# SamuelGong/FLASHE

Measured on AMD Instinct MI355X. Metric: ciphertexts/sec (enc+agg+dec), 1e7-elem vector; achieved HBM GB/s fraction, higher is better.
Workload: dtype u128

## Files before the change

flashe_amd/csrc/abi.hip:

```cpp
#include "ctx.h"
#include "blockpool.h"

#include <algorithm>
#include <cstdarg>
#include <cstdio>
#include <cstdlib>
#include <cmath>
#include <cstring>
#include <mutex>
#include <new>
#include <string>
#include <vector>

using namespace flashe;

namespace {

struct AesTables {
    uint8_t sbox[256];
    uint32_t te0[256];
    AesTables()
    {
        uint8_t alog[256], lg[256];
        uint8_t x = 1;
// ... 816 lines not shown
        idx[c] = first_idx + static_cast<uint32_t>(c);
        if (idx[c] < first_idx) return fail(ctx, FLASHE_EINVAL, "the cohort's cipher indices wrap around 2^32");
    }
    if ((rc = check_double_idx(ctx, FLASHE_SCHEME_DOUBLE, idx.data(), n_clients))) return rc;
    if (n == 0) return FLASHE_OK;
    for (int c = 0; c < n_clients; c++)
        if (!mask_dev[c] || (reinterpret_cast<uintptr_t>(mask_dev[c]) & 3u)) return fail(ctx, FLASHE_EINVAL, "vector %d: null or not 4-byte aligned", c);
    LaunchEnv env = ctx->env;
    env.elem32 = 1;
    const std::vector<const uint64_t *> none(static_cast<size_t>(n_clients), nullptr);
    return batch_shares(ctx, n_clients, [&](int v0, int nv) {
        return launch_prf_batch(env, iter, true, nv, idx.data() + v0, none.data() + v0, 1, reinterpret_cast<uint64_t *const *>(mask_dev + v0), n, n_jobs);
    });
}

int flashe_encrypt_batch_sum_u32_dev(flashe_ctx *ctx, uint32_t iter, int scheme, uint64_t n, uint32_t n_jobs, int n_vec, const uint32_t *idx,
                                     const uint32_t *const *pt_dev, uint32_t *const *ct_dev, uint32_t *sum_out_dev)
{
    CHECK_CTX(ctx);
    if (n && !sum_out_dev) return fail(ctx, FLASHE_EINVAL, "flashe_encrypt_batch_sum_u32_dev: null sum_out_dev");
    if (reinterpret_cast<uintptr_t>(sum_out_dev) & 3u) return fail(ctx, FLASHE_EINVAL, "sum_out_dev must be 4-byte aligned");
    if (n && ct_dev) { if (int rc = check_sum_apart(ctx, sum_out_dev, n_vec, pt_dev, ct_dev)) return rc; }
    if (scheme == FLASHE_SCHEME_DOUBLE && n && n_vec > 0 && n_vec <= kMaxUniformBatch && idx && pt_dev && ct_dev) {
        int rc = check_u32(ctx, n, n_jobs);
        if (rc || (rc = check_double_idx(ctx, scheme, idx, n_vec))) return rc;
        bool ok = true;
        for (int v = 0; v < n_vec && ok; v++)
            ok = pt_dev[v] && ct_dev[v] && !((reinterpret_cast<uintptr_t>(pt_dev[v]) | reinterpret_cast<uintptr_t>(ct_dev[v])) & 3u) && (v == 0 || idx[v] == idx[v - 1] + 1u);
        if (ok) {
            LaunchEnv env = ctx->env;
            env.elem32 = 1;
            std::vector<uint32_t> sidx(idx, idx + n_vec);
            sidx.push_back(idx[n_vec - 1] + 1u);
            PrfChain ch{sidx.data(), n_vec, false, 0, n, reinterpret_cast<const uint64_t *const *>(pt_dev), 1, reinterpret_cast<uint64_t *const *>(ct_dev)};
            ch.sum_out_dev = reinterpret_cast<uint64_t *>(sum_out_dev);
            const hipError_t e = launch_prf_chains(env, iter, 1, &ch, n, n_jobs);
            if (e == hipSuccess) return FLASHE_OK;
            if (e != hipErrorNotSupported) HIP_TRY(ctx, e);
        }
    }
    int rc = flashe_encrypt_batch_u32_dev(ctx, iter, scheme, n, n_jobs, n_vec, idx, pt_dev, ct_dev);
    if (rc || n == 0) return rc;
    if (n_vec == 0) { HIP_TRY(ctx, hipMemsetAsync(sum_out_dev, 0, n * 4, ctx->env.stream)); return FLASHE_OK; }
    return flashe_aggregate_elem_u32_dev(ctx, n_vec, ct_dev, n, sum_out_dev);
}

int flashe_aggregate_decrypt_u32_dev(flashe_ctx *ctx, uint32_t iter, const uint32_t *add_idx, int n_add, const uint32_t *minus_idx, int n_minus,
                                     uint64_t n, uint32_t n_jobs, uint64_t first, uint64_t count, int C, const uint32_t *const *cts_dev,
                                     void *agg_out_dev, void *out_dev, int out_elem_bytes)
{
    CHECK_CTX(ctx);
    if (C < 1 || C > kMaxOps || !cts_dev || (count && !out_dev)) return fail(ctx, FLASHE_EINVAL, "aggregate_decrypt_u32: bad arguments (C = %d, at most %d)", C, kMaxOps);
    if (out_elem_bytes != 4 && out_elem_bytes != 8) return fail(ctx, FLASHE_EINVAL, "out_elem_bytes must be 4 or 8");
    if (n_add != 1 || n_minus < 0 || n_minus > 1 || !add_idx || (n_minus && !minus_idx))
        return fail(ctx, FLASHE_EINVAL, "aggregate_decrypt_u32: one add and at most one minus prefix (widen the vectors for prefix lists)");
    int rc = check_u32(ctx, n, n_jobs);
    if (rc) return rc;
    rc = check_range(ctx, n, first, count);
    if (rc) return rc;
    if (count == 0) return FLASHE_OK;
    if ((rc = check_operands(ctx, C, cts_dev, 4))) return rc;
    const uintptr_t need = static_cast<uintptr_t>(out_elem_bytes - 1);
    if ((reinterpret_cast<uintptr_t>(out_dev) | reinterpret_cast<uintptr_t>(agg_out_dev)) & need) return fail(ctx, FLASHE_EINVAL, "outputs must be %d-byte aligned", out_elem_bytes);
    LaunchEnv env = ctx->env;
    env.elem32 = 1;
    if (C == 1 && !agg_out_dev && out_elem_bytes == 4 && n_minus == 1) {
        const uint32_t sidx[2] = {add_idx[0], minus_idx[0]};
        const uint64_t *in1 = reinterpret_cast<const uint64_t *>(cts_dev[0]);
        uint64_t *out1 = static_cast<uint64_t *>(out_dev);
        PrfChain ch{sidx, 1, false, first, count, &in1, 1, &out1};
        const hipError_t e = launch_prf_chains(env, iter, 1, &ch, n, n_jobs);
        if (e == hipSuccess) return FLASHE_OK;
        if (e != hipErrorNotSupported) HIP_TRY(ctx, e);
    }
    HIP_TRY(ctx, launch_small_reduce_decrypt(env, iter, add_idx[0], n_minus == 1, n_minus ? minus_idx[0] : 0u, n, n_jobs, first, count, C,
                                             reinterpret_cast<const uint64_t *const *>(cts_dev), static_cast<uint64_t *>(agg_out_dev),
                                             static_cast<uint64_t *>(out_dev), out_elem_bytes));
    return FLASHE_OK;
}

int flashe_aggregate_elem_u32_dev(flashe_ctx *ctx, int C, const uint32_t *const *cts_dev, uint64_t n, uint32_t *out_dev)
// ... 17 lines not shown

int flashe_widen_u32_dev(flashe_ctx *ctx, uint64_t n, const uint32_t *in_dev, uint64_t *out_dev)
{
    CHECK_CTX(ctx);
    if (n && (!in_dev || !out_dev)) return fail(ctx, FLASHE_EINVAL, "widen_u32: null vector");
    HIP_TRY(ctx, launch_widen_u32(ctx->env, n, in_dev, out_dev));
    return FLASHE_OK;
}

int flashe_narrow_u32_dev(flashe_ctx *ctx, uint64_t n, const uint64_t *in_dev, uint32_t *out_dev)
{
    CHECK_CTX(ctx);
    if (n && (!in_dev || !out_dev)) return fail(ctx, FLASHE_EINVAL, "narrow_u32: null vector");
    HIP_TRY(ctx, launch_narrow_u32(ctx->env, n, in_dev, out_dev));
    return FLASHE_OK;
}

static uint64_t *chain_dmask_begin(flashe_ctx *ctx, uint64_t count)
{
    flashe_ctx::ChainDmask &s = ctx->chain_dmask;
    s.valid = false;
    if (!ctx->chain_dmask_on || ctx->capturing || ctx->limbs != 2 || count == 0) return nullptr;
    if (ensure(ctx, s.d, vec_bytes(ctx, count)) != FLASHE_OK) {
        (void)hipGetLastError();
        ctx->err.clear();
        return nullptr;
    }
    return static_cast<uint64_t *>(s.d.p);
}

static void chain_dmask_commit(flashe_ctx *ctx, uint32_t iter, const uint32_t *idx, int n_vec, uint64_t n, uint32_t n_jobs, uint64_t first,
                               uint64_t count)
{
    flashe_ctx::ChainDmask &s = ctx->chain_dmask;
    s.iter = iter; s.key_epoch = ctx->key_epoch; s.add_idx = idx[n_vec - 1] + 1u; s.minus_idx = idx[0];
    s.n = n; s.n_jobs = n_jobs; s.first = first; s.count = count;
    s.valid = true;
}

static const uint64_t *chain_dmask_match(const flashe_ctx *ctx, uint32_t iter, const uint32_t *add_idx, int n_add, const uint32_t *minus_idx,
                                         int n_minus, uint64_t n, uint32_t n_jobs, uint64_t first, uint64_t count)
{
    const flashe_ctx::ChainDmask &s = ctx->chain_dmask;
    if (!s.valid || ctx->capturing || n_add != 1 || n_minus != 1 || count == 0) return nullptr;
    if (add_idx[0] != s.add_idx || minus_idx[0] != s.minus_idx || iter != s.iter || ctx->key_epoch != s.key_epoch || n != s.n ||
        n_jobs != s.n_jobs)
        return nullptr;
    if (first < s.first || first - s.first > s.count || count > s.count - (first - s.first)) return nullptr;
    return static_cast<const uint64_t *>(s.d.p) + (first - s.first) * 2;
}

static int encrypt_batch_sum(flashe_ctx *ctx, uint32_t iter, int scheme, uint64_t n, uint32_t n_jobs, int n_vec, const uint32_t *idx,
                             const uint64_t *const *pt_dev, int pt_limbs, uint64_t *const *ct_dev, uint64_t *sum_out_dev, uint64_t *dec_out_dev,
                             bool *dec_done)
{
    if (!sum_out_dev && n && n_vec) return fail(ctx, FLASHE_EINVAL, "flashe_encrypt_batch_sum_dev: null sum_out_dev");
    if (n_vec > 0) { if (int rc = check_double_idx(ctx, scheme, idx, n_vec)) return rc; }
    if (n && n_vec) {
        if (int rc = check_sum_aligned(ctx, sum_out_dev)) return rc;
        if (int rc = check_sum_apart(ctx, sum_out_dev, n_vec, pt_dev, ct_dev)) return rc;
    }
    if (scheme == FLASHE_SCHEME_DOUBLE && n && n_vec > 0 && idx && pt_dev && ct_dev) {
        bool ok = true;
        for (int v = 0; v < n_vec && ok; v++) ok = pt_dev[v] && ct_dev[v];
        if (ok) {
            for (int v = 0; v < n_vec; v++) {
                int rc = check_prf_args(ctx, 1, scheme, n_jobs, ct_dev[v], pt_dev[v], pt_limbs);
                if (rc) return rc;
            }
            if (dec_out_dev && ctx->chain_dec_on) {
                const hipError_t e = launch_prf_batch_sum(ctx->env, iter, n_vec, idx, pt_dev, pt_limbs, ct_dev, sum_out_dev, n, n_jobs, 0, n, nullptr,
                                                          dec_out_dev);
                if (e == hipSuccess) { *dec_done = true; return FLASHE_OK; }
                if (e != hipErrorNotSupported) HIP_TRY(ctx, e);
            }
            uint64_t *const dmask = chain_dmask_begin(ctx, n);
            const hipError_t e = launch_prf_batch_sum(ctx->env, iter, n_vec, idx, pt_dev, pt_limbs, ct_dev, sum_out_dev, n, n_jobs, 0, n, dmask);
            if (e == hipSuccess) {
                if (dmask) chain_dmask_commit(ctx, iter, idx, n_vec, n, n_jobs, 0, n);
                return FLASHE_OK;
            }
            if (e != hipErrorNotSupported) HIP_TRY(ctx, e);
        }
    }
    int rc = flashe_encrypt_batch_dev(ctx, iter, scheme, n, n_jobs, n_vec, idx, pt_dev, pt_limbs, ct_dev);
    if (rc || n == 0) return rc;
    if (n_vec == 0) { HIP_TRY(ctx, hipMemsetAsync(sum_out_dev, 0, n * ctx->limbs * 8, ctx->env.stream)); return FLASHE_OK; }
    return flashe_aggregate_elem_dev(ctx, n_vec, ct_dev, n, sum_out_dev);
}

int flashe_encrypt_batch_sum_dev(flashe_ctx *ctx, uint32_t iter, int scheme, uint64_t n, uint32_t n_jobs, int n_vec, const uint32_t *idx,
                                 const uint64_t *const *pt_dev, int pt_limbs, uint64_t *const *ct_dev, uint64_t *sum_out_dev)
{
    CHECK_CTX(ctx);
// ... 171 lines not shown
    int rc = check_range(ctx, n, first, count);
    if (rc || (rc = check_double_idx(ctx, scheme, idx, n_vec))) return rc;
    if (n_jobs == 0) return fail(ctx, FLASHE_EINVAL, "n_jobs must be >= 1");
    if (ctx->env.prf_backend != PRF_AUTO && ctx->env.prf_backend != PRF_TABLE) return fail(ctx, FLASHE_EINVAL, "encrypt_batch_range runs on the table PRF only");
    for (int v = 0; v < n_vec; v++) {
        if (count && (!pt_dev[v] || !ct_dev[v])) return fail(ctx, FLASHE_EINVAL, "null vector %d", v);
        if (sum_out_dev && (ct_dev[v] == sum_out_dev || pt_dev[v] == sum_out_dev))
            return fail(ctx, FLASHE_EINVAL, "sum_out_dev must not be one of the plaintext or ciphertext vectors");
        rc = check_prf_args(ctx, 1, scheme, n_jobs, ct_dev[v], pt_dev[v], pt_limbs);
        if (rc) return rc;
    }
    if (sum_out_dev && (rc = check_sum_aligned(ctx, sum_out_dev))) return rc;
    if (count == 0) return FLASHE_OK;
    if (n_vec == 0) { if (sum_out_dev) HIP_TRY(ctx, hipMemsetAsync(sum_out_dev, 0, vec_bytes(ctx, count), ctx->env.stream)); return FLASHE_OK; }
    if (sum_out_dev && scheme == FLASHE_SCHEME_DOUBLE) {
        uint64_t *const dmask = chain_dmask_begin(ctx, count);
        const hipError_t e = launch_prf_batch_sum(ctx->env, iter, n_vec, idx, pt_dev, pt_limbs, ct_dev, sum_out_dev, n, n_jobs, first, count, dmask);
        if (e == hipSuccess) {
            if (dmask) chain_dmask_commit(ctx, iter, idx, n_vec, n, n_jobs, first, count);
            return FLASHE_OK;
        }
        if (e != hipErrorNotSupported) HIP_TRY(ctx, e);
    }
    rc = batch_shares(ctx, n_vec, [&](int v0, int nv) {
        return launch_prf_batch_range(ctx->env, iter, scheme == FLASHE_SCHEME_DOUBLE, nv, idx + v0, pt_dev + v0, pt_limbs, ct_dev + v0, n, n_jobs,
                                      first, count);
    });
    if (rc) return rc;
    if (sum_out_dev) return flashe_aggregate_elem_dev(ctx, n_vec, ct_dev, count, sum_out_dev);
    return FLASHE_OK;
}

int flashe_decrypt_range_dev(flashe_ctx *ctx, uint32_t iter, const uint32_t *add_idx, int n_add, const uint32_t *minus_idx,
                             int n_minus, uint64_t n, uint32_t n_jobs, uint64_t first, uint64_t count,
                             const uint64_t *in_dev, uint64_t *out_dev)
{
    CHECK_CTX(ctx);
    if (count && (!in_dev || !out_dev)) return fail(ctx, FLASHE_EINVAL, "null vector");
    int rc = check_prf_args(ctx, n_add, n_minus, n_jobs, out_dev, in_dev, ctx->limbs);
    if (rc || (rc = check_range(ctx, n, first, count))) return rc;
    if (n_add == 0 && n_minus == 0) {
        HIP_TRY(ctx, launch_combine(ctx->env, count, in_dev, ctx->limbs, nullptr, nullptr, out_dev));
        return FLASHE_OK;
    }
    if (const uint64_t *d = chain_dmask_match(ctx, iter, add_idx, n_add, minus_idx, n_minus, n, n_jobs, first, count)) {
        HIP_TRY(ctx, launch_combine(ctx->env, count, in_dev, ctx->limbs, d, nullptr, out_dev));
        return FLASHE_OK;
    }
    HIP_TRY(ctx, prf_lists(ctx, iter, add_idx, n_add, minus_idx, n_minus, n, n_jobs, first, count, in_dev, ctx->limbs, out_dev));
    return FLASHE_OK;
}

int flashe_combine_dev(flashe_ctx *ctx, uint64_t n, const uint64_t *in_dev, int in_limbs, const uint64_t *add_dev,
                       const uint64_t *minus_dev, uint64_t *out_dev)
{
    CHECK_CTX(ctx);
    if (n && (!in_dev || !out_dev)) return fail(ctx, FLASHE_EINVAL, "null vector");
    if (in_limbs != 1 && in_limbs != ctx->limbs) return fail(ctx, FLASHE_EINVAL, "in_limbs must be 1 or %d", ctx->limbs);
    if (ctx->limbs == 2 && (!aligned16(out_dev) || !aligned16(add_dev) || !aligned16(minus_dev) || (in_limbs == 2 && !aligned16(in_dev))))
        return fail(ctx, FLASHE_EINVAL, "device vectors must be 16-byte aligned");
// ... 884 lines not shown
```

flashe_amd/csrc/ctx.h:

```cpp
#pragma once
#include "flashe.h"
#include "kernels.h"
#include "blockpool.h"

#include <algorithm>
#include <initializer_list>
#include <string>
#include <vector>

struct flashe_ctx {
    int device = 0;
    int device_cus = 0;
    int int_bits = 0;
    int limbs = 0;
    bool own_stream = false;
    flashe::LaunchEnv env{};
    uint32_t *te0_dev = nullptr;
    uint32_t *rkw_dev = nullptr;
    uint32_t *rkp_dev = nullptr;
    std::string err;
    struct Buf { void *p = nullptr; size_t cap = 0; };
    Buf summaries;
    Buf stream_tmp;
    Buf acc_tmp[2];
    Buf sp_ws;
    Buf bounds;
    Buf mt_ws;
    Buf draw_tab;
    Buf codec_tab;
    Buf tensor_ws;
    Buf tensor_tab;
    Buf stat_ws;
    hipEvent_t ev_foreign = nullptr;
    struct Prepared { Buf add, minus; uint64_t n = 0; bool valid = false, has_minus = false; uint32_t iter = 0, add_idx = 0, minus_idx = 0; };
    Prepared prep_enc, prep_dec;
    struct ChainDmask { Buf d; uint64_t n = 0, first = 0, count = 0; uint32_t iter = 0, key_epoch = 0, add_idx = 0, minus_idx = 0, n_jobs = 0; bool valid = false; };
    ChainDmask chain_dmask;
    bool chain_dmask_on = true;
    bool chain_dec_on = true;
    flashe_pool::StagingPool *staging = nullptr;
    bool capturing = false;
    uint32_t key_epoch = 0;
    hipEvent_t ev_copy[2] = {nullptr, nullptr};
    uint32_t *err_flag_host = nullptr;
};

namespace flashe_host {

int fail(flashe_ctx *ctx, int code, const char *fmt, ...) __attribute__((format(printf, 3, 4)));

inline size_t vec_bytes(const flashe_ctx *ctx, uint64_t n) { return static_cast<size_t>(n) * ctx->limbs * 8; }
// ... 70 lines not shown
```

flashe_amd/csrc/kernels.h:

```cpp
#pragma once
#include <hip/hip_runtime.h>
#include <stdint.h>

namespace flashe_philox { struct ClientPlan; }

namespace flashe {

struct RoundKeys { uint32_t w[60]; };

struct CodecLayer {
    uint64_t start;
    const void *x;
    double p0, p1, p2;
    int x_is_f64, pad_;
};
struct Codec {
    const void *x;
    const double *u;
    double alpha, scale, den;
    int x_is_f64, n_layers;
    double *fout;
    double ac, two_a, uden;
    const CodecLayer *layers;
    uint64_t k0;
// ... 82 lines not shown
                           uint32_t n_jobs);

struct PrfChain {
    const uint32_t *idx;
    int n_out;
    bool single;
    uint64_t first, count;
    const uint64_t *const *in_dev;
    int in_limbs;
    uint64_t *const *out_dev;
    uint64_t *sum_out_dev = nullptr;
    uint64_t *dmask_dev = nullptr;
    uint64_t *dec_out_dev = nullptr;
};
hipError_t launch_prf_chains(const LaunchEnv &env, uint32_t iter, int n_chains, const PrfChain *chains, uint64_t n, uint32_t n_jobs);

hipError_t launch_combine(const LaunchEnv &env, uint64_t n, const uint64_t *in_dev, int in_limbs,
                          const uint64_t *add_dev, const uint64_t *minus_dev, uint64_t *out_dev);

hipError_t launch_combine_batch(const LaunchEnv &env, uint64_t n, int n_vec, const uint64_t *const *in_dev, int in_limbs,
                                const uint64_t *const *add_dev, const uint64_t *const *minus_dev, uint64_t *const *out_dev);
hipError_t launch_combine_batch_sum(const LaunchEnv &env, uint64_t n, int n_vec, const uint64_t *const *in_dev, int in_limbs,
                                    const uint64_t *const *add_dev, const uint64_t *const *minus_dev, uint64_t *const *out_dev, uint64_t *sum_out_dev,
                                    const uint64_t *dec_add_dev = nullptr, const uint64_t *dec_minus_dev = nullptr, uint64_t *dec_out_dev = nullptr);

constexpr int kMaxOps = 64;
struct PtrTable { const uint64_t *p[kMaxOps]; };

hipError_t launch_small_reduce_decrypt(const LaunchEnv &env, uint32_t iter, uint32_t add_idx, bool has_minus, uint32_t minus_idx, uint64_t n,
                                       uint32_t n_jobs, uint64_t first, uint64_t count, int C, const uint64_t *const *ops, uint64_t *agg_out_dev,
// ... 209 lines not shown
```

flashe_amd/csrc/kernels.hip:

```cpp
#include "device_common.h"
#include "cohort_streams.h"
#include "cohort_cut.h"
#include <cassert>
#include <type_traits>

namespace flashe {

struct IdxLists {
    uint32_t add[kMaxIdx];
    uint32_t minus[kMaxIdx];
};

struct PrfParams {
    const uint64_t *in;
    uint64_t *out;
    const uint32_t *te0;
    uint64_t n;
    uint64_t first, count;
    uint64_t blk_first, blk_count;
    uint64_t mask_lo, mask_hi;
    uint32_t iter;
    int in_limbs;
    int n_add, n_minus;
    uint32_t n_jobs;
// ... 925 lines not shown
}

#ifndef FLASHE_FIXED32_WIDTHS
#define FLASHE_FIXED32_WIDTHS(X) X(16) X(20) X(23) X(24) X(32)
#endif
static bool fixed32_width(int b)
{
    switch (b) {
#define FLASHE_FIXED32_CASE(B) case B:
        FLASHE_FIXED32_WIDTHS(FLASHE_FIXED32_CASE)
#undef FLASHE_FIXED32_CASE
        return true;
    default: return false;
    }
}
template <int M> struct DirectPt { uint32_t v[M]; };
typedef uint32_t u32x4_a4 __attribute__((ext_vector_type(4), aligned(4)));
typedef uint32_t u32x2_a4 __attribute__((ext_vector_type(2), aligned(4)));

template <int M>
__device__ __forceinline__ DirectPt<M> direct32_load(const uint32_t *__restrict__ in, uint64_t k)
{
    DirectPt<M> r;
#pragma unroll
    for (int t = 0; t < M; t++) r.v[t] = 0u;
    if (!in) return r;
    const uint32_t *q = in + k;
    int t = 0;
#pragma unroll
    for (; t + 4 <= M; t += 4) {
// ... 131 lines not shown
#pragma unroll
    for (; t + 4 <= M; t += 4) {
        u32x4_a4 x;
        x[0] = r[t] & mask; x[1] = r[t + 1] & mask; x[2] = r[t + 2] & mask; x[3] = r[t + 3] & mask;
        *reinterpret_cast<u32x4_a4 *>(q + t) = x;
    }
    if (M - t >= 2) {
        u32x2_a4 x;
        x[0] = r[t] & mask; x[1] = r[t + 1] & mask;
        *reinterpret_cast<u32x2_a4 *>(q + t) = x;
        t += 2;
    }
    if (t < M) q[t] = r[t] & mask;
}

template <int B, bool SINGLE, class SRC = void, class OT = uint32_t, class GP = void>
__device__ __forceinline__ void small_chain_fast32(const RoundKeys &rk, const LaneRegs lr, const uint32_t *pre_lds, int sbase, int n_streams,
                                                   const uint64_t *const *in_tab, uint64_t *const *out_tab, const CtrVar &xA, const CtrVar &xB,
                                                   uint64_t kA, uint64_t kB, uint32_t *sum32, bool prio,
                                                   const uint32_t *__restrict__ te4, bool uni, uint32_t x3A, uint32_t x3B, const SRC *src = nullptr,
                                                   const GP *gaps = nullptr)
{
    constexpr bool GAPS = !std::is_void_v<GP>;
    static_assert(!GAPS || !SINGLE, "several runs are a form of the double-mask chain");
    constexpr int M = 128 / B;
    constexpr uint32_t mask = B >= 32 ? 0xffffffffu : ((1u << (B & 31)) - 1u);
    uint32_t psA[M], psB[M], accA[M], accB[M];
#pragma unroll
    for (int t = 0; t < M; t++) { psA[t] = 0u; psB[t] = 0u; accA[t] = 0u; accB[t] = 0u; }
    auto prefix_of = [&](const uint4 &v) {
        return CtrPrefix{{static_cast<uint32_t>(__builtin_amdgcn_readfirstlane(v.x)), static_cast<uint32_t>(__builtin_amdgcn_readfirstlane(v.y)),
                          static_cast<uint32_t>(__builtin_amdgcn_readfirstlane(v.z)), static_cast<uint32_t>(__builtin_amdgcn_readfirstlane(v.w))}};
    };
    uint4 pv = *reinterpret_cast<const uint4 *>(pre_lds + 4 * sbase);
    auto emit = [&](int link, const u128 SA, const u128 SB, const DirectPt<M> &dA, const DirectPt<M> &dB) {
        uint32_t csA[M], csB[M];
#pragma unroll
        for (int t = 0; t < M; t++) {
            csA[t] = static_cast<uint32_t>(SA >> (B * t));
// ... 2 lines not shown
        if (link >= 0) {
            uint32_t rA[M], rB[M];
#pragma unroll
            for (int t = 0; t < M; t++) {
                const uint32_t ua = dA.v[t] + (SINGLE ? csA[t] : psA[t] - csA[t]), ub = dB.v[t] + (SINGLE ? csB[t] : psB[t] - csB[t]);
                accA[t] += ua; accB[t] += ub;
                rA[t] = ua; rB[t] = ub;
            }
            OT *out = reinterpret_cast<OT *>(out_tab[link]);
            direct32_put<M>(out + kA, rA, mask);
            direct32_put<M>(out + kB, rB, mask);
        }
#pragma unroll
        for (int t = 0; t < M; t++) { psA[t] = csA[t]; psB[t] = csB[t]; }
    };
    for (int c = 0; c < n_streams; c++) {
        const CtrPrefix pre = prefix_of(pv);
        pv = *reinterpret_cast<const uint4 *>(pre_lds + 4 * (sbase + (c + 1 < n_streams ? c + 1 : c)));
        int link = SINGLE ? c : c - 1;
        if constexpr (GAPS) link = cohort_stream_link(*gaps, c);
        DirectPt<M> dA{}, dB{};
        if (link >= 0) {
            if constexpr (std::is_void_v<SRC>) {
                const uint32_t *in = reinterpret_cast<const uint32_t *>(in_tab[link]);
                dA = direct32_load<M>(in, kA);
                dB = direct32_load<M>(in, kB);
            } else {
                dA = src->template block<M>(link, kA, 0);
                dB = src->template block<M>(link, kB, 1);
            }
// ... 3 lines not shown
            const CtrUniform UA = ctr_uniform(rk, te4, pre, x3A), UB = ctr_uniform(rk, te4, pre, x3B);
            ctr_round2(lr, pre.u[0], xA.v[0], UA, s[0]);
            ctr_round2(lr, pre.u[0], xB.v[0], UB, s[1]);
            aes256_rounds<2, 3>(rk, lr, s, prio);
        } else {
            ctr_round1(pre, xA, s[0]);
            ctr_round1(pre, xB, s[1]);
            aes256_rounds<2, 2>(rk, lr, s, prio);
        }
        emit(link, words_to_u128(s[0]), words_to_u128(s[1]), dA, dB);
    }
    if (sum32) {
        direct32_put<M>(sum32 + kA, accA, mask);
        direct32_put<M>(sum32 + kB, accB, mask);
    }
}

__device__ __forceinline__ u128 slot_diff(u128 prev, u128 cur, u128 top, int b)
{
    if (b == 64) {
        const uint64_t lo = static_cast<uint64_t>(prev) - static_cast<uint64_t>(cur), hi = static_cast<uint64_t>(prev >> 64) - static_cast<uint64_t>(cur >> 64);
        return (static_cast<u128>(hi) << 64) | lo;
    }
    return ((prev | top) - (cur & ~top)) ^ ((prev ^ ~cur) & top);
}

template <bool PAIR, class ET = uint64_t, int B = 0>
__global__ __launch_bounds__(kSmallThreads) void prf_small_chain_kernel(const RoundKeys rk, const SmallChainTable tb, int n_chains, const SmallParams p)
{
    constexpr bool COHORT = false, GAPS = false;
    const CohortCodec cc{};
    const CohortGaps cg{};
#include "prf_small_chain_body.inc"
}

template <int B>
__global__ __launch_bounds__(kSmallThreads) void prf_small_cohort_kernel(const RoundKeys rk, const SmallChainTable tb, int n_chains, const SmallParams p,
                                                                          const CohortCodec cc)
{
    constexpr bool PAIR = true, COHORT = true, GAPS = false;
    using ET = uint32_t;
    const CohortGaps cg{};
#include "prf_small_chain_body.inc"
}

template <int B>
__global__ __launch_bounds__(kSmallThreads) void prf_small_cohort_runs_kernel(const RoundKeys rk, const SmallChainTable tb, int n_chains, const SmallParams p,
                                                                               const CohortCodec cc, const CohortGaps cg)
{
    constexpr bool PAIR = true, COHORT = true, GAPS = true;
    using ET = uint32_t;
#include "prf_small_chain_body.inc"
}

struct SparseCohortTail {
    const double *zzz;
    uint64_t *zeros;
    const double *u_n;
    uint64_t u_stride, n;
    double alpha, scale, den;
    int f64, n_clients;
};
template <int B>
__global__ __launch_bounds__(kSmallThreads) void prf_small_sparse_cohort_kernel(const RoundKeys rk, const SmallChainTable tb, int n_chains, const SmallParams p,
                                                                                 const CohortCodec cc, const SparseCohortTail tail)
{
    constexpr bool PAIR = true, COHORT = true, GAPS = false;
    using ET = uint64_t;
    const CohortGaps cg{};
    if (blockIdx.x == 0 && threadIdx.x < static_cast<unsigned>(tail.n_clients)) {
        const int c = threadIdx.x;
        const double v = tail.zzz[c], u = tail.u_n[static_cast<uint64_t>(c) * tail.u_stride];
        const uint64_t q = tail.f64 ? quantize_one<double>(v, tail.alpha, tail.scale, tail.den, u)
                                    : quantize_one<float>(static_cast<float>(v), static_cast<float>(tail.alpha), static_cast<float>(tail.scale),
                                                          static_cast<float>(tail.den), u);
        tail.zeros[c] = q;
        tb.out[c][tail.n] = q;
    }
#include "prf_small_chain_body.inc"
}


template <int CB, int EPL>
__global__ __launch_bounds__(kSmallThreads) void small_reduce_decrypt_kernel(const RoundKeys rk, const SmallParams p, uint32_t add_idx, uint32_t minus_idx,
// ... 1036 lines not shown
{
    int prio = env.elem32 ? (!p.no_fixed_width && fixed32_width(env.b) && (env.b != 20 || longest <= 1)) : (p.m <= 4 && !p.no_direct);
    { static const int v = FLASHE_TUNE_ENV("FLASHE_SMALL_PRIO") ? atoi(FLASHE_TUNE_ENV("FLASHE_SMALL_PRIO")) : -1; if (v >= 0) prio = v; }
    return prio;
}

static hipError_t launch_small_chains(const LaunchEnv &env, uint32_t iter, int n_chains, const PrfChain *chains, uint64_t n, uint32_t n_jobs)
{
    if (env.codec || n >= (1ull << 32) || n == 0) return hipErrorNotSupported;
    SmallParams p = small_params_of(env, iter, n, n_jobs);
    bool summed = false;
    for (int i = 0; i < n_chains; i++) summed |= chains[i].sum_out_dev != nullptr;
    if (summed && !(env.elem32 && !p.no_fixed_width && fixed32_width(env.b) && n_chains == 1 && !chains[0].single &&
                    chains[0].n_out <= kMaxLinks))
        return hipErrorNotSupported;
    if (env.elem32) {
        if (env.b > 32) return hipErrorInvalidValue;
        p.no_direct = 1;
    }
    int longest = 0;
    for (int i = 0; i < n_chains; i++) longest = std::max(longest, chains[i].n_out);
    p.swp_prio = small_swp_prio(env, p, longest);
    struct Piece { const PrfChain *ch; int l0, l1; uint64_t blk_first, blk_count; };
    std::vector<Piece> pieces;
    uint64_t total_blocks = 0;
    for (int i = 0; i < n_chains; i++) {
        const PrfChain &c = chains[i];
        if (c.count == 0 || c.n_out == 0) continue;
        if (c.in_dev && c.in_limbs != 1) return hipErrorInvalidValue;
        const uint64_t bf = block_of(c.first, n, n_jobs, p.m), bc = block_of(c.first + c.count - 1, n, n_jobs, p.m) - bf + 1;
// ... 37 lines not shown
            for (int l = 0; l < len; l++) {
                tb.in[links + l] = c.in_dev ? c.in_dev[pc.l0 + l] : nullptr;
                tb.out[links + l] = c.out_dev[pc.l0 + l];
            }
            tb.sum_out[nc] = c.sum_out_dev;
            const uint64_t t = (pc.blk_count + tile - 1) / tile;
            wend += t * static_cast<uint64_t>(ns);
            tb.wend[nc] = wend;
            tiles += t;
            links += len; streams += ns; nc++;
        }
        const uint64_t cus = static_cast<uint64_t>(env.num_cus);
        const int grid = static_cast<int>(tiles < cus ? tiles : cus);
        if (env.elem32) {
            const int fixed = (pair && !p.no_fixed_width) ? env.b : 0;
            switch (fixed) {
#define FLASHE_FIXED32(B) case B: hipLaunchKernelGGL((prf_small_chain_kernel<true, uint32_t, B>), dim3(grid), dim3(kSmallThreads), 0, env.stream, env.rk, tb, nc, p); break;
                FLASHE_FIXED32_WIDTHS(FLASHE_FIXED32)
#undef FLASHE_FIXED32
            default:
                if (pair) hipLaunchKernelGGL((prf_small_chain_kernel<true, uint32_t>), dim3(grid), dim3(kSmallThreads), 0, env.stream, env.rk, tb, nc, p);
                else hipLaunchKernelGGL((prf_small_chain_kernel<false, uint32_t>), dim3(grid), dim3(kSmallThreads), 0, env.stream, env.rk, tb, nc, p);
            }
        } else if (pair && env.b == 64 && !p.no_fixed_width && !p.no_direct)
            hipLaunchKernelGGL((prf_small_chain_kernel<true, uint64_t, 64>), dim3(grid), dim3(kSmallThreads), 0, env.stream, env.rk, tb, nc, p);
        else if (pair) hipLaunchKernelGGL((prf_small_chain_kernel<true>), dim3(grid), dim3(kSmallThreads), 0, env.stream, env.rk, tb, nc, p);
        else hipLaunchKernelGGL((prf_small_chain_kernel<false>), dim3(grid), dim3(kSmallThreads), 0, env.stream, env.rk, tb, nc, p);
        const hipError_t e = hipGetLastError();
        if (e != hipSuccess) return e;
    }
// ... 268 lines not shown
```

flashe_amd/csrc/prf_small_chain_body.inc:

```
    static_assert(!COHORT || (PAIR && B != 0 && B <= 32), "the cohort front end rides on the paired chain at a compile-time width");
    static_assert(!GAPS || (COHORT && sizeof(ET) == 4), "several runs of indices are a form of the summed compact cohort chain");
    (void)cc;
    (void)cg;
    constexpr bool LIMB_OUT = COHORT && sizeof(ET) == 8;
    static_assert(B == 0 || (PAIR && ((sizeof(ET) == 4 && B <= 32) || (sizeof(ET) == 8 && (B == 64 || LIMB_OUT)))), "compile-time widths: the paired kernel, compact layout or int_bits 64");
    constexpr uint32_t WAVES = kSmallThreads / 64, TILE = PAIR ? 128u : 64u;
    constexpr int MB = B ? 128 / B : 1;
    __shared__ uint32_t tab[kTabWords];
    __shared__ uint32_t scratch[(kSmallThreads / 64) * 256 + 8];
    __shared__ __attribute__((aligned(16))) uint32_t pre_lds[(kMaxLinks + kMaxChains) * 4];
    __shared__ uint64_t d_tlo[kMaxChains], d_cend[kMaxChains];
    const uint32_t iter = p.iter + p.te0[kIterShiftWord];
    fill_tables(tab, p.te0);
    const LaneRegs lr = lane_regs(tab);
    {
        const int last = n_chains - 1;
        const int n_streams = GAPS ? cg.n_streams : tb.sbase[last] + tb.len[last] + ((tb.flags[last] & 1) ? 0 : 1);
        for (int s = threadIdx.x; s < n_streams; s += kSmallThreads) {
            const CtrPrefix c = ctr_prefix(rk, lr, iter, tb.idx[s], 0u);
            *reinterpret_cast<uint4 *>(pre_lds + 4 * s) = make_uint4(c.u[0], c.u[1], c.u[2], c.u[3]);
        }
        if (threadIdx.x < static_cast<unsigned>(n_chains)) {
            const int i = threadIdx.x;
            const uint64_t Wt = tb.wend[last], cw = i ? tb.wend[i - 1] : 0;
// ... 28 lines not shown
    const uint32_t lane = threadIdx.x & 63u;
    const uint32_t wave = static_cast<uint32_t>(__builtin_amdgcn_readfirstlane(threadIdx.x >> 6));
    uint32_t *row0 = scratch + wave * 256;
    const u128 top = (static_cast<u128>(p.top_hi) << 64) | p.top_lo;
    const bool direct = p.m <= 4 && !p.no_direct;
    const bool walk32 = p.b <= 32 && !direct && p.no_direct != 2;
    const uint32_t wblk0 = lane / m32, wo0 = (lane - wblk0 * m32) * static_cast<uint32_t>(p.b);
    const uint64_t Ng = uniform64(d_cend[n_chains - 1]);
    int cur = 0;
    uint64_t cbeg = 0;
    for (uint64_t q = wave; q < Ng; q += WAVES) {
        while (q >= uniform64(d_cend[cur])) cbeg = uniform64(d_cend[cur++]);
        const uint64_t first = tb.first[cur], range_end = first + tb.count[cur], blk_count = tb.blk_count[cur];
        const uint64_t Bw = (uniform64(d_tlo[cur]) + (q - cbeg)) * TILE;
        const int link0 = tb.link0[cur], sbase = tb.sbase[cur];
        const bool single = tb.flags[cur] & 1;
        const int n_streams = GAPS ? cg.n_streams : tb.len[cur] + (single ? 0 : 1);
        const bool vA = Bw + lane < blk_count, vB = PAIR && Bw + 64u + lane < blk_count;
        uint64_t j0A = 0, j0B = 0;
        int cntA = 0, cntB = 0;
        uint32_t ctrA = 0, ctrB = 0;
        small_block_params(static_cast<uint32_t>(tb.blk_first[cur] + (vA ? Bw + lane : 0)), nb1_32, nb0_32, d32, r32, m32, p, &j0A, &cntA, &ctrA);
        if (PAIR) small_block_params(static_cast<uint32_t>(tb.blk_first[cur] + (vB ? Bw + 64u + lane : 0)), nb1_32, nb0_32, d32, r32, m32, p, &j0B, &cntB, &ctrB);
        const CtrVar xA = ctr_var(rk, lr, ctrA);
        CtrVar xB{};
        if (PAIR) xB = ctr_var(rk, lr, ctrB);
        uint64_t e0A = 0, e0B = 0;
        bool fastA = false, fastB = false;
        if (walk32) {
            e0A = uniform64(j0A);
            fastA = __ballot(vA && cntA == p.m) == ~0ull && e0A >= first && e0A + 64u * m64 <= range_end;
// ... 30 lines not shown
                                 (bA & 255u) <= 192u && (bB & 255u) <= 192u;
                if constexpr (LIMB_OUT) {
                    const CohortDirect csrc{cc, tb.in + link0, link0, {layA, layB}};
                    small_chain_fast32<B, true, CohortDirect, uint64_t>(rk, lr, pre_lds, sbase, n_streams, tb.in + link0, tb.out + link0, xA, xB, j0A - first, j0B - first,
                                                                        nullptr, p.swp_prio != 0, p.te0, uni, bA ^ rk.w[3], bB ^ rk.w[3], &csrc);
                    continue;
                } else if constexpr (GAPS) {
                    const CohortDirect csrc{cc, tb.in + link0, link0, {layA, layB}};
                    small_chain_fast32<B, false, CohortDirect, uint32_t, CohortGaps>(rk, lr, pre_lds, sbase, n_streams, tb.in + link0, tb.out + link0, xA, xB, j0A - first, j0B - first,
                                                                                     sum32, p.swp_prio != 0, p.te0, false, 0u, 0u, &csrc, &cg);
                    continue;
                } else if constexpr (COHORT) {
                    const CohortDirect csrc{cc, tb.in + link0, link0, {layA, layB}};
                    small_chain_fast32<B, false>(rk, lr, pre_lds, sbase, n_streams, tb.in + link0, tb.out + link0, xA, xB, j0A - first, j0B - first, sum32, p.swp_prio != 0,
                                                 p.te0, uni, bA ^ rk.w[3], bB ^ rk.w[3], &csrc);
                    continue;
                }
                if (single) small_chain_fast32<B, true>(rk, lr, pre_lds, sbase, n_streams, tb.in + link0, tb.out + link0, xA, xB, j0A - first, j0B - first, sum32, p.swp_prio != 0,
                                                        p.te0, uni, bA ^ rk.w[3], bB ^ rk.w[3]);
                else small_chain_fast32<B, false>(rk, lr, pre_lds, sbase, n_streams, tb.in + link0, tb.out + link0, xA, xB, j0A - first, j0B - first, sum32, p.swp_prio != 0,
                                                  p.te0, uni, bA ^ rk.w[3], bB ^ rk.w[3]);
                continue;
            }
        }
        if (PAIR) {
            for (int c = 0; c < n_streams; c++) {
                const CtrPrefix pre = load_prefix(pre_lds, sbase + c);
                const int link = GAPS ? cohort_stream_link(cg, c) : single ? c : c - 1;
                WalkPt ptA{}, ptB{};
                DirectPt<MB> dA{}, dB{};
// ... 64 lines not shown
                        if (fastA) small_walk32(row0, lane, e0A, DA, ptA, ein, eout, first, p, wblk0, wo0);
                        else small_walk(row0, lane, vA, cntA, j0A, DA, ein, eout, first, range_end, p);
                        if (fastB) small_walk32(row0, lane, e0B, DB, ptB, ein, eout, first, p, wblk0, wo0);
                        else small_walk(row0, lane, vB, cntB, j0B, DB, ein, eout, first, range_end, p);
                    }
                }
                prevA = SA; prevB = SB;
            }
            if constexpr (B != 0 && B != 64) {
                if (sum32) {
                    constexpr uint32_t bmask = B >= 32 ? 0xffffffffu : ((1u << (B & 31)) - 1u);
                    if (fastA) direct32_put<MB>(sum32 + (j0A - first), accA, bmask);
                    if (fastB) direct32_put<MB>(sum32 + (j0B - first), accB, bmask);
                }
            }
        } else {
            for (int c = 0; c < n_streams; c += 2) {
                const bool has1 = c + 1 < n_streams;
                const CtrPrefix pre0 = load_prefix(pre_lds, sbase + c), pre1 = load_prefix(pre_lds, sbase + (has1 ? c + 1 : c));
                const int l0 = single ? c : c - 1;
                WalkPt pt0{}, pt1{};
                if (fastA && l0 >= 0) pt0 = small_walk32_load(reinterpret_cast<const ET *>(tb.in[link0 + l0]), e0A, first, lane, m32);
                if (fastA && has1) pt1 = small_walk32_load(reinterpret_cast<const ET *>(tb.in[link0 + l0 + 1]), e0A, first, lane, m32);
                uint32_t s[2][4];
                ctr_round1(pre0, xA, s[0]);
                ctr_round1(pre1, xA, s[1]);
                aes256_rounds<2, 2>(rk, lr, s, true);
                const u128 S0 = words_to_u128(s[0]), S1 = words_to_u128(s[1]);
                if (l0 >= 0) {
                    const u128 D = single ? S0 : slot_diff(prevA, S0, top, p.b);
// ... 19 lines not shown
```

Baseline: 75.82 billion.

## Emit decrypt mask from the u32 summed encrypt chain and reuse it in decrypt

Extends the cached decrypt-mask mechanism to the compact 32-bit summed encrypt chain. A new kernel variant writes the combined add-minus mask while encrypting. The u32 aggregate-decrypt path then applies that mask with a plain elementwise subtract instead of re-running AES for the mask streams. This trades an extra mask write, plus a matching read in decrypt, for dropping the PRF recomputation. It also adds register and LDS-stash pressure to the fused encrypt kernel.

```diff
diff --git a/flashe_amd/csrc/abi.hip b/flashe_amd/csrc/abi.hip
--- a/flashe_amd/csrc/abi.hip
+++ b/flashe_amd/csrc/abi.hip
@@ -854,6 +854,41 @@
     });
 }
 
+static void *chain_dmask_begin(flashe_ctx *ctx, uint64_t count, int elem_bytes)
+{
+    flashe_ctx::ChainDmask &s = ctx->chain_dmask;
+    s.valid = false;
+    if (!ctx->chain_dmask_on || ctx->capturing || count == 0) return nullptr;
+    if (elem_bytes == 16 ? ctx->limbs != 2 : !(elem_bytes == 4 && small_chain_dmask_width(ctx->int_bits))) return nullptr;
+    if (ensure(ctx, s.d, static_cast<size_t>(count) * static_cast<size_t>(elem_bytes)) != FLASHE_OK) {
+        (void)hipGetLastError();
+        ctx->err.clear();
+        return nullptr;
+    }
+    return s.d.p;
+}
+
+static void chain_dmask_commit(flashe_ctx *ctx, uint32_t iter, const uint32_t *idx, int n_vec, uint64_t n, uint32_t n_jobs, uint64_t first,
+                               uint64_t count, int elem_bytes)
+{
+    flashe_ctx::ChainDmask &s = ctx->chain_dmask;
+    s.iter = iter; s.key_epoch = ctx->key_epoch; s.add_idx = idx[n_vec - 1] + 1u; s.minus_idx = idx[0];
+    s.n = n; s.n_jobs = n_jobs; s.first = first; s.count = count; s.elem_bytes = elem_bytes;
+    s.valid = true;
+}
+
+static const void *chain_dmask_match(const flashe_ctx *ctx, uint32_t iter, const uint32_t *add_idx, int n_add, const uint32_t *minus_idx,
+                                     int n_minus, uint64_t n, uint32_t n_jobs, uint64_t first, uint64_t count, int elem_bytes)
+{
+    const flashe_ctx::ChainDmask &s = ctx->chain_dmask;
+    if (!s.valid || ctx->capturing || n_add != 1 || n_minus != 1 || count == 0 || elem_bytes != s.elem_bytes) return nullptr;
+    if (add_idx[0] != s.add_idx || minus_idx[0] != s.minus_idx || iter != s.iter || ctx->key_epoch != s.key_epoch || n != s.n ||
+        n_jobs != s.n_jobs)
+        return nullptr;
+    if (first < s.first || first - s.first > s.count || count > s.count - (first - s.first)) return nullptr;
+    return static_cast<const char *>(s.d.p) + (first - s.first) * static_cast<uint64_t>(elem_bytes);
+}
+
 int flashe_encrypt_batch_sum_u32_dev(flashe_ctx *ctx, uint32_t iter, int scheme, uint64_t n, uint32_t n_jobs, int n_vec, const uint32_t *idx,
                                      const uint32_t *const *pt_dev, uint32_t *const *ct_dev, uint32_t *sum_out_dev)
 {
@@ -874,8 +909,12 @@
             sidx.push_back(idx[n_vec - 1] + 1u);
             PrfChain ch{sidx.data(), n_vec, false, 0, n, reinterpret_cast<const uint64_t *const *>(pt_dev), 1, reinterpret_cast<uint64_t *const *>(ct_dev)};
             ch.sum_out_dev = reinterpret_cast<uint64_t *>(sum_out_dev);
+            ch.dmask_dev = static_cast<uint64_t *>(chain_dmask_begin(ctx, n, 4));
             const hipError_t e = launch_prf_chains(env, iter, 1, &ch, n, n_jobs);
-            if (e == hipSuccess) return FLASHE_OK;
+            if (e == hipSuccess) {
+                if (ch.dmask_dev) chain_dmask_commit(ctx, iter, idx, n_vec, n, n_jobs, 0, n, 4);
+                return FLASHE_OK;
+            }
             if (e != hipErrorNotSupported) HIP_TRY(ctx, e);
         }
     }
@@ -905,6 +944,11 @@
     LaunchEnv env = ctx->env;
     env.elem32 = 1;
     if (C == 1 && !agg_out_dev && out_elem_bytes == 4 && n_minus == 1) {
+        if (const void *d = chain_dmask_match(ctx, iter, add_idx, n_add, minus_idx, n_minus, n, n_jobs, first, count, 4)) {
+            const uint32_t *const ops[2] = {cts_dev[0], static_cast<const uint32_t *>(d)};
+            HIP_TRY(ctx, launch_aggregate_elem_u32(env, 2, ops, count, static_cast<uint32_t *>(out_dev)));
+            return FLASHE_OK;
+        }
         const uint32_t sidx[2] = {add_idx[0], minus_idx[0]};
         const uint64_t *in1 = reinterpret_cast<const uint64_t *>(cts_dev[0]);
         uint64_t *out1 = static_cast<uint64_t *>(out_dev);
@@ -952,40 +996,6 @@
     if (n && (!in_dev || !out_dev)) return fail(ctx, FLASHE_EINVAL, "narrow_u32: null vector");
     HIP_TRY(ctx, launch_narrow_u32(ctx->env, n, in_dev, out_dev));
     return FLASHE_OK;
-}
-
-static uint64_t *chain_dmask_begin(flashe_ctx *ctx, uint64_t count)
-{
-    flashe_ctx::ChainDmask &s = ctx->chain_dmask;
-    s.valid = false;
-    if (!ctx->chain_dmask_on || ctx->capturing || ctx->limbs != 2 || count == 0) return nullptr;
-    if (ensure(ctx, s.d, vec_bytes(ctx, count)) != FLASHE_OK) {
-        (void)hipGetLastError();
-        ctx->err.clear();
-        return nullptr;
-    }
-    return static_cast<uint64_t *>(s.d.p);
-}
-
-static void chain_dmask_commit(flashe_ctx *ctx, uint32_t iter, const uint32_t *idx, int n_vec, uint64_t n, uint32_t n_jobs, uint64_t first,
-                               uint64_t count)
-{
-    flashe_ctx::ChainDmask &s = ctx->chain_dmask;
-    s.iter = iter; s.key_epoch = ctx->key_epoch; s.add_idx = idx[n_vec - 1] + 1u; s.minus_idx = idx[0];
-    s.n = n; s.n_jobs = n_jobs; s.first = first; s.count = count;
-    s.valid = true;
-}
-
-static const uint64_t *chain_dmask_match(const flashe_ctx *ctx, uint32_t iter, const uint32_t *add_idx, int n_add, const uint32_t *minus_idx,
-                                         int n_minus, uint64_t n, uint32_t n_jobs, uint64_t first, uint64_t count)
-{
-    const flashe_ctx::ChainDmask &s = ctx->chain_dmask;
-    if (!s.valid || ctx->capturing || n_add != 1 || n_minus != 1 || count == 0) return nullptr;
-    if (add_idx[0] != s.add_idx || minus_idx[0] != s.minus_idx || iter != s.iter || ctx->key_epoch != s.key_epoch || n != s.n ||
-        n_jobs != s.n_jobs)
-        return nullptr;
-    if (first < s.first || first - s.first > s.count || count > s.count - (first - s.first)) return nullptr;
-    return static_cast<const uint64_t *>(s.d.p) + (first - s.first) * 2;
 }
 
 static int encrypt_batch_sum(flashe_ctx *ctx, uint32_t iter, int scheme, uint64_t n, uint32_t n_jobs, int n_vec, const uint32_t *idx,
@@ -1012,10 +1022,10 @@
                 if (e == hipSuccess) { *dec_done = true; return FLASHE_OK; }
                 if (e != hipErrorNotSupported) HIP_TRY(ctx, e);
             }
-            uint64_t *const dmask = chain_dmask_begin(ctx, n);
+            uint64_t *const dmask = static_cast<uint64_t *>(chain_dmask_begin(ctx, n, 16));
             const hipError_t e = launch_prf_batch_sum(ctx->env, iter, n_vec, idx, pt_dev, pt_limbs, ct_dev, sum_out_dev, n, n_jobs, 0, n, dmask);
             if (e == hipSuccess) {
-                if (dmask) chain_dmask_commit(ctx, iter, idx, n_vec, n, n_jobs, 0, n);
+                if (dmask) chain_dmask_commit(ctx, iter, idx, n_vec, n, n_jobs, 0, n, 16);
                 return FLASHE_OK;
             }
             if (e != hipErrorNotSupported) HIP_TRY(ctx, e);
@@ -1217,10 +1227,10 @@
     if (count == 0) return FLASHE_OK;
     if (n_vec == 0) { if (sum_out_dev) HIP_TRY(ctx, hipMemsetAsync(sum_out_dev, 0, vec_bytes(ctx, count), ctx->env.stream)); return FLASHE_OK; }
     if (sum_out_dev && scheme == FLASHE_SCHEME_DOUBLE) {
-        uint64_t *const dmask = chain_dmask_begin(ctx, count);
+        uint64_t *const dmask = static_cast<uint64_t *>(chain_dmask_begin(ctx, count, 16));
         const hipError_t e = launch_prf_batch_sum(ctx->env, iter, n_vec, idx, pt_dev, pt_limbs, ct_dev, sum_out_dev, n, n_jobs, first, count, dmask);
         if (e == hipSuccess) {
-            if (dmask) chain_dmask_commit(ctx, iter, idx, n_vec, n, n_jobs, first, count);
+            if (dmask) chain_dmask_commit(ctx, iter, idx, n_vec, n, n_jobs, first, count, 16);
             return FLASHE_OK;
         }
         if (e != hipErrorNotSupported) HIP_TRY(ctx, e);
@@ -1246,7 +1256,7 @@
         HIP_TRY(ctx, launch_combine(ctx->env, count, in_dev, ctx->limbs, nullptr, nullptr, out_dev));
         return FLASHE_OK;
     }
-    if (const uint64_t *d = chain_dmask_match(ctx, iter, add_idx, n_add, minus_idx, n_minus, n, n_jobs, first, count)) {
+    if (const uint64_t *d = static_cast<const uint64_t *>(chain_dmask_match(ctx, iter, add_idx, n_add, minus_idx, n_minus, n, n_jobs, first, count, 16))) {
         HIP_TRY(ctx, launch_combine(ctx->env, count, in_dev, ctx->limbs, d, nullptr, out_dev));
         return FLASHE_OK;
     }
diff --git a/flashe_amd/csrc/ctx.h b/flashe_amd/csrc/ctx.h
--- a/flashe_amd/csrc/ctx.h
+++ b/flashe_amd/csrc/ctx.h
@@ -34,7 +34,7 @@
     hipEvent_t ev_foreign = nullptr;
     struct Prepared { Buf add, minus; uint64_t n = 0; bool valid = false, has_minus = false; uint32_t iter = 0, add_idx = 0, minus_idx = 0; };
     Prepared prep_enc, prep_dec;
-    struct ChainDmask { Buf d; uint64_t n = 0, first = 0, count = 0; uint32_t iter = 0, key_epoch = 0, add_idx = 0, minus_idx = 0, n_jobs = 0; bool valid = false; };
+    struct ChainDmask { Buf d; uint64_t n = 0, first = 0, count = 0; uint32_t iter = 0, key_epoch = 0, add_idx = 0, minus_idx = 0, n_jobs = 0; int elem_bytes = 0; bool valid = false; };
     ChainDmask chain_dmask;
     bool chain_dmask_on = true;
     bool chain_dec_on = true;
diff --git a/flashe_amd/csrc/kernels.h b/flashe_amd/csrc/kernels.h
--- a/flashe_amd/csrc/kernels.h
+++ b/flashe_amd/csrc/kernels.h
@@ -120,6 +120,7 @@
     uint64_t *dec_out_dev = nullptr;
 };
 hipError_t launch_prf_chains(const LaunchEnv &env, uint32_t iter, int n_chains, const PrfChain *chains, uint64_t n, uint32_t n_jobs);
+bool small_chain_dmask_width(int b);
 
 hipError_t launch_combine(const LaunchEnv &env, uint64_t n, const uint64_t *in_dev, int in_limbs,
                           const uint64_t *add_dev, const uint64_t *minus_dev, uint64_t *out_dev);
diff --git a/flashe_amd/csrc/kernels.hip b/flashe_amd/csrc/kernels.hip
--- a/flashe_amd/csrc/kernels.hip
+++ b/flashe_amd/csrc/kernels.hip
@@ -963,6 +963,13 @@
     default: return false;
     }
 }
+bool small_chain_dmask_width(int b)
+{
+    switch (b) {
+    case 16: case 20: case 23: case 24: case 32: return fixed32_width(b);
+    default: return false;
+    }
+}
 template <int M> struct DirectPt { uint32_t v[M]; };
 typedef uint32_t u32x4_a4 __attribute__((ext_vector_type(4), aligned(4)));
 typedef uint32_t u32x2_a4 __attribute__((ext_vector_type(2), aligned(4)));
@@ -1124,15 +1131,16 @@
     if (t < M) q[t] = r[t] & mask;
 }
 
-template <int B, bool SINGLE, class SRC = void, class OT = uint32_t, class GP = void>
+template <int B, bool SINGLE, class SRC = void, class OT = uint32_t, class GP = void, bool DM = false>
 __device__ __forceinline__ void small_chain_fast32(const RoundKeys &rk, const LaneRegs lr, const uint32_t *pre_lds, int sbase, int n_streams,
                                                    const uint64_t *const *in_tab, uint64_t *const *out_tab, const CtrVar &xA, const CtrVar &xB,
                                                    uint64_t kA, uint64_t kB, uint32_t *sum32, bool prio,
                                                    const uint32_t *__restrict__ te4, bool uni, uint32_t x3A, uint32_t x3B, const SRC *src = nullptr,
-                                                   const GP *gaps = nullptr)
+                                                   const GP *gaps = nullptr, uint32_t *dmask32 = nullptr, uint32_t *stash = nullptr)
 {
     constexpr bool GAPS = !std::is_void_v<GP>;
     static_assert(!GAPS || !SINGLE, "several runs are a form of the double-mask chain");
+    static_assert(!DM || (!SINGLE && !GAPS && std::is_void_v<SRC> && sizeof(OT) == 4), "the decrypt mask: the plain summed double-mask chain");
     constexpr int M = 128 / B;
     constexpr uint32_t mask = B >= 32 ? 0xffffffffu : ((1u << (B & 31)) - 1u);
     uint32_t psA[M], psB[M], accA[M], accB[M];
@@ -1165,6 +1173,31 @@
 #pragma unroll
         for (int t = 0; t < M; t++) { psA[t] = csA[t]; psB[t] = csB[t]; }
     };
+    [[maybe_unused]] u128 firstB = 0;
+    if constexpr (DM) {
+        {
+            const CtrPrefix pre = prefix_of(pv);
+            pv = *reinterpret_cast<const uint4 *>(pre_lds + 4 * (sbase + (1 < n_streams ? 1 : 0)));
+            uint32_t s[2][4];
+            ctr_round1(pre, xA, s[0]);
+            ctr_round1(pre, xB, s[1]);
+            aes256_rounds<2, 2>(rk, lr, s, prio);
+            *reinterpret_cast<uint4 *>(stash) = make_uint4(s[0][0], s[0][1], s[0][2], s[0][3]);
+            firstB = words_to_u128(s[1]);
+            emit(-1, words_to_u128(s[0]), firstB, DirectPt<M>{}, DirectPt<M>{});
+        }
+        for (int c = 1; c < n_streams; c++) {
+            const CtrPrefix pre = prefix_of(pv);
+            pv = *reinterpret_cast<const uint4 *>(pre_lds + 4 * (sbase + (c + 1 < n_streams ? c + 1 : c)));
+            const uint32_t *in = reinterpret_cast<const uint32_t *>(in_tab[c - 1]);
+            const DirectPt<M> dA = direct32_load<M>(in, kA), dB = direct32_load<M>(in, kB);
+            uint32_t s[2][4];
+            ctr_round1(pre, xA, s[0]);
+            ctr_round1(pre, xB, s[1]);
+            aes256_rounds<2, 2>(rk, lr, s, prio);
+            emit(c - 1, words_to_u128(s[0]), words_to_u128(s[1]), dA, dB);
+        }
+    } else
     for (int c = 0; c < n_streams; c++) {
         const CtrPrefix pre = prefix_of(pv);
         pv = *reinterpret_cast<const uint4 *>(pre_lds + 4 * (sbase + (c + 1 < n_streams ? c + 1 : c)));
@@ -1198,6 +1231,19 @@
         direct32_put<M>(sum32 + kA, accA, mask);
         direct32_put<M>(sum32 + kB, accB, mask);
     }
+    if constexpr (DM) {
+        const uint4 fv = *reinterpret_cast<const uint4 *>(stash);
+        const uint32_t fw[4] = {fv.x, fv.y, fv.z, fv.w};
+        const u128 firstA = words_to_u128(fw);
+        uint32_t mA[M], mB[M];
+#pragma unroll
+        for (int t = 0; t < M; t++) {
+            mA[t] = psA[t] - static_cast<uint32_t>(firstA >> (B * t));
+            mB[t] = psB[t] - static_cast<uint32_t>(firstB >> (B * t));
+        }
+        direct32_put<M>(dmask32 + kA, mA, mask);
+        direct32_put<M>(dmask32 + kB, mB, mask);
+    }
 }
 
 __device__ __forceinline__ u128 slot_diff(u128 prev, u128 cur, u128 top, int b)
@@ -1212,7 +1258,19 @@
 template <bool PAIR, class ET = uint64_t, int B = 0>
 __global__ __launch_bounds__(kSmallThreads) void prf_small_chain_kernel(const RoundKeys rk, const SmallChainTable tb, int n_chains, const SmallParams p)
 {
-    constexpr bool COHORT = false, GAPS = false;
+    constexpr bool COHORT = false, GAPS = false, DMASK = false;
+    const CohortCodec cc{};
+    const CohortGaps cg{};
+    uint32_t *const dmask = nullptr;
+#include "prf_small_chain_body.inc"
+}
+
+template <int B>
+__global__ __launch_bounds__(kSmallThreads) void prf_small_dmask_kernel(const RoundKeys rk, const SmallChainTable tb, int n_chains, const SmallParams p,
+                                                                         uint32_t *dmask)
+{
+    constexpr bool PAIR = true, COHORT = false, GAPS = false, DMASK = true;
+    using ET = uint32_t;
     const CohortCodec cc{};
     const CohortGaps cg{};
 #include "prf_small_chain_body.inc"
@@ -1222,9 +1280,10 @@
 __global__ __launch_bounds__(kSmallThreads) void prf_small_cohort_kernel(const RoundKeys rk, const SmallChainTable tb, int n_chains, const SmallParams p,
                                                                           const CohortCodec cc)
 {
-    constexpr bool PAIR = true, COHORT = true, GAPS = false;
+    constexpr bool PAIR = true, COHORT = true, GAPS = false, DMASK = false;
     using ET = uint32_t;
     const CohortGaps cg{};
+    uint32_t *const dmask = nullptr;
 #include "prf_small_chain_body.inc"
 }
 
@@ -1232,8 +1291,9 @@
 __global__ __launch_bounds__(kSmallThreads) void prf_small_cohort_runs_kernel(const RoundKeys rk, const SmallChainTable tb, int n_chains, const SmallParams p,
                                                                                const CohortCodec cc, const CohortGaps cg)
 {
-    constexpr bool PAIR = true, COHORT = true, GAPS = true;
+    constexpr bool PAIR = true, COHORT = true, GAPS = true, DMASK = false;
     using ET = uint32_t;
+    uint32_t *const dmask = nullptr;
 #include "prf_small_chain_body.inc"
 }
 
@@ -1249,9 +1309,10 @@
 __global__ __launch_bounds__(kSmallThreads) void prf_small_sparse_cohort_kernel(const RoundKeys rk, const SmallChainTable tb, int n_chains, const SmallParams p,
                                                                                  const CohortCodec cc, const SparseCohortTail tail)
 {
-    constexpr bool PAIR = true, COHORT = true, GAPS = false;
+    constexpr bool PAIR = true, COHORT = true, GAPS = false, DMASK = false;
     using ET = uint64_t;
     const CohortGaps cg{};
+    uint32_t *const dmask = nullptr;
     if (blockIdx.x == 0 && threadIdx.x < static_cast<unsigned>(tail.n_clients)) {
         const int c = threadIdx.x;
         const double v = tail.zzz[c], u = tail.u_n[static_cast<uint64_t>(c) * tail.u_stride];
@@ -2318,6 +2379,8 @@
     if (summed && !(env.elem32 && !p.no_fixed_width && fixed32_width(env.b) && n_chains == 1 && !chains[0].single &&
                     chains[0].n_out <= kMaxLinks))
         return hipErrorNotSupported;
+    for (int i = 0; i < n_chains; i++) if (chains[i].dmask_dev && !(summed && small_chain_dmask_width(env.b))) return hipErrorInvalidValue;
+    uint32_t *const dmask32 = summed ? reinterpret_cast<uint32_t *>(chains[0].dmask_dev) : nullptr;
     if (env.elem32) {
         if (env.b > 32) return hipErrorInvalidValue;
         p.no_direct = 1;
@@ -2385,6 +2448,14 @@
         const int grid = static_cast<int>(tiles < cus ? tiles : cus);
         if (env.elem32) {
             const int fixed = (pair && !p.no_fixed_width) ? env.b : 0;
+            if (dmask32) {
+                switch (fixed) {
+#define FLASHE_FIXED32(B) case B: hipLaunchKernelGGL((prf_small_dmask_kernel<B>), dim3(grid), dim3(kSmallThreads), 0, env.stream, env.rk, tb, nc, p, dmask32); break;
+                    FLASHE_FIXED32_WIDTHS(FLASHE_FIXED32)
+#undef FLASHE_FIXED32
+                default: return hipErrorInvalidValue;
+                }
+            } else
             switch (fixed) {
 #define FLASHE_FIXED32(B) case B: hipLaunchKernelGGL((prf_small_chain_kernel<true, uint32_t, B>), dim3(grid), dim3(kSmallThreads), 0, env.stream, env.rk, tb, nc, p); break;
                 FLASHE_FIXED32_WIDTHS(FLASHE_FIXED32)
diff --git a/flashe_amd/csrc/prf_small_chain_body.inc b/flashe_amd/csrc/prf_small_chain_body.inc
--- a/flashe_amd/csrc/prf_small_chain_body.inc
+++ b/flashe_amd/csrc/prf_small_chain_body.inc
@@ -1,4 +1,6 @@
     static_assert(!COHORT || (PAIR && B != 0 && B <= 32), "the cohort front end rides on the paired chain at a compile-time width");
+    static_assert(!DMASK || (PAIR && !COHORT && !GAPS && sizeof(ET) == 4 && B != 0 && B <= 32), "the decrypt mask rides on the plain compact paired chain at a compile-time width");
+    (void)dmask;
     static_assert(!GAPS || (COHORT && sizeof(ET) == 4), "several runs of indices are a form of the summed compact cohort chain");
     (void)cc;
     (void)cg;
@@ -66,7 +68,7 @@
         const uint64_t first = tb.first[cur], range_end = first + tb.count[cur], blk_count = tb.blk_count[cur];
         const uint64_t Bw = (uniform64(d_tlo[cur]) + (q - cbeg)) * TILE;
         const int link0 = tb.link0[cur], sbase = tb.sbase[cur];
-        const bool single = tb.flags[cur] & 1;
+        const bool single = !DMASK && (tb.flags[cur] & 1);
         const int n_streams = GAPS ? cg.n_streams : tb.len[cur] + (single ? 0 : 1);
         const bool vA = Bw + lane < blk_count, vB = PAIR && Bw + 64u + lane < blk_count;
         uint64_t j0A = 0, j0B = 0;
@@ -127,6 +129,10 @@
                     const CohortDirect csrc{cc, tb.in + link0, link0, {layA, layB}};
                     small_chain_fast32<B, false>(rk, lr, pre_lds, sbase, n_streams, tb.in + link0, tb.out + link0, xA, xB, j0A - first, j0B - first, sum32, p.swp_prio != 0,
                                                  p.te0, uni, bA ^ rk.w[3], bB ^ rk.w[3], &csrc);
+                    continue;
+                } else if constexpr (DMASK) {
+                    small_chain_fast32<B, false, void, uint32_t, void, true>(rk, lr, pre_lds, sbase, n_streams, tb.in + link0, tb.out + link0, xA, xB, j0A - first, j0B - first,
+                                                                             sum32, p.swp_prio != 0, p.te0, uni, bA ^ rk.w[3], bB ^ rk.w[3], nullptr, nullptr, dmask, row0 + 4 * lane);
                     continue;
                 }
                 if (single) small_chain_fast32<B, true>(rk, lr, pre_lds, sbase, n_streams, tb.in + link0, tb.out + link0, xA, xB, j0A - first, j0B - first, sum32, p.swp_prio != 0,
@@ -221,6 +227,29 @@
                     if (fastB) direct32_put<MB>(sum32 + (j0B - first), accB, bmask);
                 }
             }
+            if constexpr (DMASK) {
+                constexpr uint32_t bmask = B >= 32 ? 0xffffffffu : ((1u << (B & 31)) - 1u);
+                uint32_t s0[2][4];
+                {
+                    const CtrPrefix pre = load_prefix(pre_lds, sbase);
+                    ctr_round1(pre, xA, s0[0]);
+                    ctr_round1(pre, xB, s0[1]);
+                    aes256_rounds<2, 2>(rk, lr, s0, p.swp_prio != 0);
+                }
+                const u128 firstA = words_to_u128(s0[0]), firstB = words_to_u128(s0[1]);
+                if (fastA) {
+                    uint32_t mA[MB];
+#pragma unroll
+                    for (int t = 0; t < MB; t++) mA[t] = static_cast<uint32_t>(prevA >> (B * t)) - static_cast<uint32_t>(firstA >> (B * t));
+                    direct32_put<MB>(dmask + (j0A - first), mA, bmask);
+                } else small_walk<uint32_t>(row0, lane, vA, cntA, j0A, slot_diff(prevA, firstA, top, p.b), static_cast<const uint32_t *>(nullptr), dmask, first, range_end, p);
+                if (fastB) {
+                    uint32_t mB[MB];
+#pragma unroll
+                    for (int t = 0; t < MB; t++) mB[t] = static_cast<uint32_t>(prevB >> (B * t)) - static_cast<uint32_t>(firstB >> (B * t));
+                    direct32_put<MB>(dmask + (j0B - first), mB, bmask);
+                } else small_walk<uint32_t>(row0, lane, vB, cntB, j0B, slot_diff(prevB, firstB, top, p.b), static_cast<const uint32_t *>(nullptr), dmask, first, range_end, p);
+            }
         } else {
             for (int c = 0; c < n_streams; c += 2) {
                 const bool has1 = c + 1 < n_streams;
```

New measurement: 75.79 billion. About the same (-0.0%).
